# LJacksonPan/RaTrack

Measured on AMD Instinct MI355X. Metric: radar frame-pairs/sec (backbone forward, eval) at B=64,N=256 per GPU, higher is better.
Workload: dtype f32 (2xfp16 split MFMA: three fp16 products per fp32 product, fp32 accumulate, power-of-two scales per matrix and position); 1 GPU; Track4D.backbone forward, B=64 frame-pairs x N=256 points per GPU, S=512 centroids, eval-mode BN, random-init weights, hipGraph=True, batches in flight=4; global_batch=64, parallelism=replicas x1 (no collective on the forward path)

## Files before the change

### ratrack_amd/csrc/fused_split.hip

```cpp
#include "rtk_common.h"
#include "rtk_fused.h"
#include "split_mfma.h"

namespace {

#ifndef SP_NW
#define SP_NW 4
#endif
#ifndef SP_F
#define SP_F 32
#endif
constexpr int CV_F = 32;

__global__ __launch_bounds__(256) void pack_split_kernel(int cout, int cin, const float *__restrict__ w, int transposed, u4v *__restrict__ out,
                                                         float *__restrict__ inv_scale) {
    __shared__ unsigned s_m[4];
    float m = 0.f;
    const f4 *w4 = reinterpret_cast<const f4 *>(w);
    for (int i = threadIdx.x; i < cout * cin / 4; i += 256) {
        const f4 t = w4[i];
        m = __builtin_fmaxf(__builtin_fmaxf(m, __builtin_fabsf(t.x)), __builtin_fabsf(t.y));
        m = __builtin_fmaxf(__builtin_fmaxf(m, __builtin_fabsf(t.z)), __builtin_fabsf(t.w));
    }
    unsigned mb = __float_as_uint(m);
#pragma unroll
    for (int d = 32; d >= 1; d >>= 1) { const unsigned o = __shfl_xor(mb, d, 64); mb = o > mb ? o : mb; }
    if ((threadIdx.x & 63) == 0) s_m[threadIdx.x >> 6] = mb;
    __syncthreads();
    mb = max(max(s_m[0], s_m[1]), max(s_m[2], s_m[3]));
    const LaneScale sc = lane_scale_of(mb);
    if (blockIdx.x == 0 && threadIdx.x == 0) *inv_scale = sc.inv;
    const int VB = cout / 32, slot = blockIdx.x * 256 + threadIdx.x;
    if (slot >= (cin / 16) * VB * 64) return;
    const int lane = slot & 63, v = (slot >> 6) % VB, s = (slot >> 6) / VB, hh = lane >> 5, i = lane & 31;
    const int o = 32 * v + i, c0 = 32 * (s >> 1) + 16 * (s & 1) + 4 * hh;
    f4 x0, x1;
    if (transposed) {
#pragma unroll
        for (int r = 0; r < 4; ++r) { x0[r] = w[(size_t)(c0 + r) * cout + o]; x1[r] = w[(size_t)(c0 + 8 + r) * cout + o]; }
    } else {
        const float *row = w + (size_t)o * cin + c0;
        x0 = *reinterpret_cast<const f4 *>(row); x1 = *reinterpret_cast<const f4 *>(row + 8);
    }
    u4v b[2];
    split2(x0, x1, sc.s, b);
#pragma unroll
    for (int p = 0; p < 2; ++p) out[((size_t)(s * VB + v) * 2 + p) * 64 + lane] = b[p];
}

__device__ __forceinline__ f4 leaky_med4(f4 t, float inf) {
    const f4 u = t * 0.1f;
    return (f4){__builtin_amdgcn_fmed3f(t.x, u.x, inf), __builtin_amdgcn_fmed3f(t.y, u.y, inf), __builtin_amdgcn_fmed3f(t.z, u.z, inf),
                __builtin_amdgcn_fmed3f(t.w, u.w, inf)};
}
__device__ __forceinline__ f4 scale_bias4(f4 a, float c, f4 b) { return __builtin_elementwise_fma(a, (f4){c, c, c, c}, b); }

__global__ __launch_bounds__(64 * SP_NW) __attribute__((amdgpu_waves_per_eu(1, 1)))
void split_mlp2_kernel(int positions, const float *__restrict__ x, const f4 *__restrict__ blob, const float *__restrict__ wsc,
                       const float *__restrict__ bias1, const float *__restrict__ bias2, float *__restrict__ y) {
    const float kinf = rtk_hidden_inf();
    __shared__ __attribute__((aligned(16))) f4 s_w[2 * SP_F * 64];
    const int lane = threadIdx.x & 63, wave = __builtin_amdgcn_readfirstlane(threadIdx.x >> 6), hh = lane >> 5, col = lane & 31;
    constexpr int NF = 2 * SPLIT_NF;
    WStreamA<SP_NW, SP_F, NF> ws;
    ws.start_parts(blob, s_w, wave, lane);
    const float wi1 = ldc(wsc), wi2 = ldc(wsc + 1);
    const int tiles = (positions + 32 * SP_NW - 1) / (32 * SP_NW);
    for (int T = blockIdx.x; T < tiles; T += gridDim.x) {
        asm volatile("" ::: "memory");
        const long pos = (long)T * 32 * SP_NW + 32 * wave + col;
        const bool valid = pos < positions;
        const float *xr = x + (valid ? pos : (long)positions - 1) * 256 + 4 * hh;
        f4 h[32], bq[2][8];
#pragma unroll
        for (int i = 0; i < 32; ++i) h[i] = *reinterpret_cast<const f4 *>(xr + 8 * i);
        f16v acc[SPLIT_VB];
        LaneScale sc = lane_scale32(h);
        split_layer<0>(ws, h, sc.s, acc, BiasSide{bias1 + 4 * hh, bq});
        float c = sc.inv * wi1;
        split_epilogue(acc, bias1 + 4 * hh, bq, [&](int e, f4 a, f4 b) { h[e] = leaky_med4(scale_bias4(a, c, b), kinf); });
        sc = lane_scale32(h);
        split_layer<SPLIT_NF>(ws, h, sc.s, acc, BiasSide{bias2 + 4 * hh, bq});
        ws.sync();
        c = sc.inv * wi2;
        float *yr = y + pos * 256 + 4 * hh;
        split_epilogue(acc, bias2 + 4 * hh, bq, [&](int e, f4 a, f4 b) {
            if (valid) *reinterpret_cast<f4 *>(yr + 8 * e) = leaky_med4(scale_bias4(a, c, b), kinf);
        });
    }
    ws.finish();
}

struct CvSplitParams {
    int samples, n1, n2, gx;
    const float *xyz1, *xyz2;
    const int64_t *knn;
    const float *p1, *p2;
    const float *st;
    const float *wd;
    const f4 *blob;
    const float *wsc;
    const float *bias2, *bias3;
    WnSplit wn;
    float *out;
    int out_pitch;
    float *amax;
    float *sv1, *sv2, *sv3;
    uint2 *mk1, *mk2;
};

__device__ __forceinline__ void split_sign_masks(const f4 (&a)[32], uint2 (&m)[2]) {
    m[0] = m[1] = make_uint2(0u, 0u);
#pragma unroll
    for (int v = 0; v < SPLIT_VB; ++v)
#pragma unroll
        for (int q = 0; q < 4; ++q)
#pragma unroll
            for (int r = 0; r < 4; ++r) {
                const unsigned bit = (a[4 * v + q][r] > 0.f ? 1u : 0u) << (4 * ((2 * v + (q >> 1)) & 7) + r);
                if (v < 4) m[q & 1].x |= bit; else m[q & 1].y |= bit;
            }
}
__device__ __forceinline__ unsigned split_mask_bits(const uint2 (&m)[2], int v, int q) {
    return ((v < 4 ? m[q & 1].x : m[q & 1].y) >> (4 * ((2 * v + (q >> 1)) & 7))) & 15u;
}

__device__ __forceinline__ f4 *cv_at(float *base, unsigned byte_off) { return reinterpret_cast<f4 *>(reinterpret_cast<char *>(base) + byte_off); }
__device__ __forceinline__ const f4 *cv_at(const float *base, unsigned byte_off) {
    return reinterpret_cast<const f4 *>(reinterpret_cast<const char *>(base) + byte_off);
}

struct WnBlock {
    f16v bias;
    float w[4];
};
__device__ __forceinline__ WnBlock wn_block(const WnSplit &W, int v, int hh, int col) {
    WnBlock k;
    k.bias = split_bias(W.bc, v, hh);
    const int ch = 32 * v + col;
    const float *wr = W.wc + ((ch >> 4) * 64 + (ch & 15)) * 4;
#pragma unroll
    for (int st = 0; st < 4; ++st) {
        const int kk = 2 * st + hh;
        k.w[st] = ldc(wr + 64 * (kk >> 2) + (kk & 3));
    }
    return k;
}
__device__ __forceinline__ f16v wn_pre(const WnBlock &k, int hh, const float (&t2)[8]) {
    f16v w = k.bias;
#pragma unroll
    for (int st = 0; st < 4; ++st) w = mfma_f32x2(k.w[st], hh ? t2[2 * st + 1] : t2[2 * st], w);
    return w;
}

#ifndef CV_LDS_HIDDEN
#define CV_LDS_HIDDEN 1
#endif
#ifndef CV_WN_AHEAD
#define CV_WN_AHEAD 2
#endif
struct CvConsts {
    float wd[SPLIT_VB * 2 * 64];
    float wc[SPLIT_VB * 4 * 64];
    float bc[256], bias2[256], bias3[256];
#if CV_LDS_HIDDEN
    float hid[128];
#endif
};
static_assert(sizeof(CvConsts) == 15 * 1024 + (CV_LDS_HIDDEN ? 512 : 0), "4 + 8 + 3 KiB (+ the hidden layers)");
struct CvConstsFill {
    f4 wd, wc[2], bias;
    float hid;
};
__device__ __forceinline__ CvConstsFill cv_consts_load(const float *wd, const WnSplit &W, const float *bias2, const float *bias3, int wave, int lane) {
    CvConstsFill k;
    const int t = wave * 64 + lane;
    k.wd = ldc4(wd + 4 * t);
#pragma unroll
    for (int n = 0; n < 2; ++n) {
        const int u = 256 * n + t;
        k.wc[n] = ldc4(W.wc + (u >> 5) * 256 + ((u >> 4) & 1) * 64 + (u & 15) * 4);
    }
    const float *bs = wave == 0 ? W.bc : wave == 1 ? bias2 : bias3;
    k.bias = ldc4(bs + 4 * lane);
#if CV_LDS_HIDDEN
    {
        const int u = t < 32 ? 0 : t - 32, o = u >> 3, c = u & 7;
        const float *hs = t < 32 ? W.wa + 16 * (t >> 3) + (t & 7) : t < 96 ? W.wb + (16 * (c >> 2) + o) * 4 + (c & 3) : W.bb + (t < 104 ? t - 96 : 0);
        k.hid = ldc(hs);
    }
#endif
    return k;
}
__device__ __forceinline__ void cv_consts_store(CvConsts &C, const CvConstsFill &k, int wave, int lane) {
    const int t = wave * 64 + lane;
    {
        const int g = t >> 4, m = (t >> 2) & 3;
        *reinterpret_cast<f4 *>(C.wd + ((g >> 1) * 2 + (m >> 1)) * 64 + (m & 1) * 32 + (g & 1) * 16 + 4 * (t & 3)) = k.wd;
    }
#pragma unroll
    for (int n = 0; n < 2; ++n) {
        const int u = 256 * n + t, g = u >> 5, kq = (u >> 4) & 1, c15 = u & 15;
#pragma unroll
        for (int k3 = 0; k3 < 4; ++k3)
            C.wc[((g >> 1) * 4 + 2 * kq + (k3 >> 1)) * 64 + (k3 & 1) * 32 + (g & 1) * 16 + c15] = k.wc[n][k3];
    }
    if (wave < 3) *reinterpret_cast<f4 *>((wave == 0 ? C.bc : wave == 1 ? C.bias2 : C.bias3) + 4 * lane) = k.bias;
#if CV_LDS_HIDDEN
    if (t < 104) C.hid[t] = k.hid;
#endif
}
#if CV_LDS_HIDDEN
__device__ __forceinline__ void wn_hidden_lds(const CvConsts &C, float dx, float dy, float dz, float (&t2)[8]) {
    float t1[8];
#pragma unroll
    for (int o = 0; o < 8; ++o) {
        float a = __fmaf_rn(C.hid[o], dx, 0.f);
        a = __fmaf_rn(C.hid[8 + o], dy, a);
        a = __fmaf_rn(C.hid[16 + o], dz, a);
        t1[o] = fmaxf(__fadd_rn(a, C.hid[24 + o]), 0.f);
    }
#pragma unroll
    for (int o = 0; o < 8; ++o) {
        float a = C.hid[96 + o];
#pragma unroll
        for (int c = 0; c < 8; ++c) a = __fmaf_rn(C.hid[32 + 8 * o + c], t1[c], a);
        t2[o] = fmaxf(a, 0.f);
    }
}
#endif
__device__ __forceinline__ WnBlock wn_block_lds(const CvConsts &C, int v, int hh, int lane) {
    WnBlock k;
#pragma unroll
    for (int q = 0; q < 4; ++q) {
        const f4 t = *reinterpret_cast<const f4 *>(C.bc + 32 * v + 8 * q + 4 * hh);
        k.bias[4 * q] = t.x; k.bias[4 * q + 1] = t.y; k.bias[4 * q + 2] = t.z; k.bias[4 * q + 3] = t.w;
    }
#pragma unroll
    for (int st = 0; st < 4; ++st) k.w[st] = C.wc[(4 * v + st) * 64 + lane];
    return k;
}

constexpr int CV_ROWS_F4 = 32 * 32;
struct CvRowsRequest {
    const char *p2;
    f4 *rows;
    int nbrow;
    unsigned lanepart;
    int sub;
    __device__ __forceinline__ CvRowsRequest(const float *p2_, f4 *rows_, int nbrow_, int half, int lane)
        : p2(reinterpret_cast<const char *>(p2_)), rows(rows_), nbrow(nbrow_), lanepart(512u * half + (unsigned)(((lane & 31) ^ (lane >> 5)) << 4)), sub(lane >> 5) {}
    template <int T>
    __device__ __forceinline__ void one() const {
        const int r0 = __builtin_amdgcn_readlane(nbrow, 2 * T), r1 = __builtin_amdgcn_readlane(nbrow, 2 * T + 1);
        const unsigned off = ((unsigned)(sub ? r1 : r0) << 10) + (lanepart ^ (unsigned)(((2 * T) & 15) << 4));
        __builtin_amdgcn_global_load_lds((const __attribute__((address_space(1))) void *)(p2 + off),
                                         (__attribute__((address_space(3))) void *)(rows + T * 64), 16, 0, 0);
    }
    template <int... T>
    __device__ __forceinline__ void all(std::integer_sequence<int, T...>) const { (one<T>(), ...); }
};
template <int HALF>
__device__ __forceinline__ void cv_rows_request(const float *p2, int nbrow, f4 *rows, int lane) {
    asm volatile("s_waitcnt lgkmcnt(0)" ::: "memory");
    CvRowsRequest(p2, rows, nbrow, HALF, lane).all(std::make_integer_sequence<int, 16>{});
}
template <bool SAVE>
struct CvLayer2Side {
    StoreRowsSide st;
    CvRowsRequest rq;
    template <int GI>
    __device__ __forceinline__ void at(const f4 (&h)[32]) const {
        if constexpr (SAVE) st.template at<GI>(h);
        constexpr int per_chunk = CV_F / SPLIT_GF, ig = split_issue_groups(CV_F), g = GI % per_chunk, n = (GI / per_chunk) * ig + g;
        if constexpr (g < ig && 3 * n < 16) {
            rq.template one<3 * n>();
            if constexpr (3 * n + 1 < 16) rq.template one<3 * n + 1>();
            if constexpr (3 * n + 2 < 16) rq.template one<3 * n + 2>();
        }
    }
};
template <int HALF>
__device__ __forceinline__ void cv_rows_read(const f4 *rows, int col, int hh, f4 (&h)[32]) {
#pragma unroll
    for (int e = 0; e < 16; ++e) h[16 * HALF + e] = rows[col * 32 + ((2 * e + hh) ^ (col & 15))];
}
template <int K>
__device__ __forceinline__ f4 add_row_bcast(const f4 q, const f4 r) {
    f4 o;
    asm("s_nop 1\n"
        "v_add_f32_dpp %0, %4, %8 row_newbcast:%12 row_mask:0xf bank_mask:0xf\n"
        "v_add_f32_dpp %1, %5, %9 row_newbcast:%12 row_mask:0xf bank_mask:0xf\n"
        "v_add_f32_dpp %2, %6, %10 row_newbcast:%12 row_mask:0xf bank_mask:0xf\n"
        "v_add_f32_dpp %3, %7, %11 row_newbcast:%12 row_mask:0xf bank_mask:0xf"
        : "=&v"(o.x), "=&v"(o.y), "=&v"(o.z), "=&v"(o.w)
        : "v"(q.x), "v"(q.y), "v"(q.z), "v"(q.w), "v"(r.x), "v"(r.y), "v"(r.z), "v"(r.w), "n"(K));
    return o;
}
template <int K>
__device__ __forceinline__ f4 mul_row_bcast(const f4 q, const f4 r) {
    f4 o;
    asm("s_nop 1\n"
        "v_mul_f32_dpp %0, %4, %8 row_newbcast:%12 row_mask:0xf bank_mask:0xf\n"
        "v_mul_f32_dpp %1, %5, %9 row_newbcast:%12 row_mask:0xf bank_mask:0xf\n"
        "v_mul_f32_dpp %2, %6, %10 row_newbcast:%12 row_mask:0xf bank_mask:0xf\n"
        "v_mul_f32_dpp %3, %7, %11 row_newbcast:%12 row_mask:0xf bank_mask:0xf"
        : "=&v"(o.x), "=&v"(o.y), "=&v"(o.z), "=&v"(o.w)
        : "v"(q.x), "v"(q.y), "v"(q.z), "v"(q.w), "v"(r.x), "v"(r.y), "v"(r.z), "v"(r.w), "n"(K));
    return o;
}
__device__ __forceinline__ f4 add4_rn(const f4 a, const f4 b) {
    return (f4){__fadd_rn(a.x, b.x), __fadd_rn(a.y, b.y), __fadd_rn(a.z, b.z), __fadd_rn(a.w, b.w)};
}
template <int V0, int V1, bool LDSC>
__device__ __forceinline__ void cv_layer1_blocks(const CvSplitParams &P, const CvConsts &C, const f4 q0, const f4 q1, float b0, float b1, int hh, int col, float kinf, f4 (&h)[32]) {
    static_assert(V1 <= 8, "eight 32-channel blocks");
    auto block = [&](auto vc) {
        constexpr int v = decltype(vc)::value;
        f16v c;
        auto slot = [&](auto qc) {
            constexpr int q = decltype(qc)::value, e = 4 * v + q;
            const f4 t = add_row_bcast<e & 15>(e < 16 ? q0 : q1, h[e]);
            c[4 * q] = t.x; c[4 * q + 1] = t.y; c[4 * q + 2] = t.z; c[4 * q + 3] = t.w;
        };
        slot(std::integral_constant<int, 0>{}); slot(std::integral_constant<int, 1>{});
        slot(std::integral_constant<int, 2>{}); slot(std::integral_constant<int, 3>{});
        float a0, a1;
        if constexpr (LDSC) {
            a0 = C.wd[(2 * v) * 64 + 32 * hh + col]; a1 = C.wd[(2 * v + 1) * 64 + 32 * hh + col];
        } else {
            const int ch = 32 * v + col;
            const float *wr = P.wd + (ch >> 4) * 64 + (ch & 15);
            a0 = ldc(wr + 16 * hh); a1 = ldc(wr + 16 * (2 + hh));
        }
        c = mfma_f32x2(a0, b0, c);
        c = mfma_f32x2(a1, b1, c);
#pragma unroll
        for (int q = 0; q < 4; ++q) h[4 * v + q] = leaky_med4((f4){c[4 * q], c[4 * q + 1], c[4 * q + 2], c[4 * q + 3]}, kinf);
    };
    block(std::integral_constant<int, V0>{}); block(std::integral_constant<int, V0 + 1>{});
    block(std::integral_constant<int, V0 + 2>{}); block(std::integral_constant<int, V0 + 3>{});
}

#ifndef CV_FWD_VGPRS
#define CV_FWD_VGPRS 448
#endif
template <bool SAVE, bool LDSC = true>
__global__ __launch_bounds__(64 * SP_NW) __attribute__((amdgpu_waves_per_eu(1, 1), amdgpu_num_vgpr(CV_FWD_VGPRS)))
void cost_volume_split_kernel(const CvSplitParams P) {
    const float kinf = rtk_hidden_inf();
    __shared__ __attribute__((aligned(16))) f4 s_w[2 * CV_F * 64];
    __shared__ __attribute__((aligned(16))) f4 s_rows[SP_NW * CV_ROWS_F4];
    __shared__ __attribute__((aligned(16))) CvConsts s_c;
    const int lane = threadIdx.x & 63, wave = __builtin_amdgcn_readfirstlane(threadIdx.x >> 6), hh = lane >> 5, col = lane & 31, pp = col >> 4,
              j = col & 15;
    f4 *rows = s_rows + wave * CV_ROWS_F4;
    constexpr int PPW = 2 * SP_NW;
    const int groups = (P.n1 + PPW - 1) / PPW;
    const bool flat = P.gx > 0;
    const int xcd = blockIdx.x & 7, t0 = flat ? (int)(blockIdx.x >> 3) : (int)blockIdx.x, tstep = flat ? P.gx >> 3 : (int)gridDim.x;
    const int ntiles = flat ? (P.samples >> 3) * groups : groups;
    auto locate = [&](int t, int &b_, int &G_) {
        if (flat) { const int sk = t / groups; b_ = sk * 8 + xcd; G_ = t - sk * groups; }
        else { b_ = blockIdx.y; G_ = t; }
    };
    int b, bx;
    locate(t0 < ntiles ? t0 : 0, b, bx);
    WStreamA<SP_NW, CV_F, 2 * SPLIT_NF> ws;
    CvConstsFill cfill;
    if constexpr (LDSC) cfill = cv_consts_load(P.wd, P.wn, P.bias2, P.bias3, wave, lane);
    ws.start_parts(P.blob, s_w, wave, lane);
    if constexpr (LDSC) {
        cv_consts_store(s_c, cfill, wave, lane);
        __syncthreads();
    }
    const float *bias2 = (LDSC ? s_c.bias2 : P.bias2) + 4 * hh, *bias3 = (LDSC ? s_c.bias3 : P.bias3) + 4 * hh;
    auto wnb = [&](int v) {
        if constexpr (LDSC) return wn_block_lds(s_c, v, hh, lane);
        else return wn_block(P.wn, v, hh, col);
    };
    const float wi2 = ldc(P.wsc), wi3 = ldc(P.wsc + 1);
    int pt = bx * PPW + 2 * wave + pp;
    bool valid = pt < P.n1;
    long i = (long)b * P.n1 + (valid ? pt : P.n1 - 1);
    long nb = 0;
    float dx = 0.f, dy = 0.f, dz = 0.f;
    f4 q0 = {0.f, 0.f, 0.f, 0.f}, q1 = q0;
    if (t0 < ntiles) {
        nb = (long)b * P.n2 + (long)P.knn[i * 16 + j];
        cv_rows_request<0>(P.p2, (int)nb, rows, lane);
        q0 = ldc4(P.p1 + i * 256 + 4 * hh + 8 * j); q1 = ldc4(P.p1 + i * 256 + 4 * hh + 8 * (16 + j));
        if (P.st) { q0 = add4_rn(q0, ldc4(P.st + b * 256 + 4 * hh + 8 * j)); q1 = add4_rn(q1, ldc4(P.st + b * 256 + 4 * hh + 8 * (16 + j))); }
        dx = __fsub_rn(P.xyz2[nb * 3], P.xyz1[i * 3]); dy = __fsub_rn(P.xyz2[nb * 3 + 1], P.xyz1[i * 3 + 1]);
        dz = __fsub_rn(P.xyz2[nb * 3 + 2], P.xyz1[i * 3 + 2]);
    }
    for (int t = t0; t < ntiles; t += tstep) {
        asm volatile("" ::: "memory");
        const bool more = t + tstep < ntiles;
        int bn, Gn;
        locate(more ? t + tstep : t, bn, Gn);
        const int ptn = Gn * PPW + 2 * wave + pp;
        const bool validn = ptn < P.n1;
        const long in_ = (long)bn * P.n1 + (validn ? ptn : P.n1 - 1);
        long knn_next = 0;
        if (more) knn_next = (long)P.knn[in_ * 16 + j];
        f4 h[32];
        float t2[8];
        {
            const float b0 = hh ? dy : dx, b1 = hh ? 0.f : dz;
            cv_rows_read<0>(rows, col, hh, h);
            cv_rows_request<1>(P.p2, (int)nb, rows, lane);
            cv_layer1_blocks<0, 4, LDSC>(P, s_c, q0, q1, b0, b1, hh, col, kinf, h);
#if CV_LDS_HIDDEN
            if constexpr (LDSC && !SAVE) wn_hidden_lds(s_c, dx, dy, dz, t2);
            else
#endif
                wn_hidden(P.wn, dx, dy, dz, t2);
            __builtin_amdgcn_sched_barrier(0);
            cv_rows_read<1>(rows, col, hh, h);
            cv_layer1_blocks<4, 8, LDSC>(P, s_c, q0, q1, b0, b1, hh, col, kinf, h);
        }
        const long nbn = (long)bn * P.n2 + knn_next;
        const long pos = i * 16 + j;
        const unsigned ro = (unsigned)pos * 1024u + 16u * hh;
        if (SAVE && valid) {
            uint2 m[2];
            split_sign_masks(h, m);
            P.mk1[pos * 4 + hh] = m[0];
            P.mk1[pos * 4 + 2 + hh] = m[1];
        }
        f16v acc[SPLIT_VB];
        f4 bq[2][8];
        LaneScale sc = lane_scale32(h);
        if (SAVE && P.amax) tensor_amax_update(P.amax, sc.mb);
        split_layer<0>(ws, h, sc.s, acc, SidePair<CvLayer2Side<SAVE>, BiasSide>{{StoreRowsSide{P.sv1, ro, valid}, CvRowsRequest(P.p2, rows, (int)nbn, 0, lane)},
                                                                              BiasSide{bias2, bq}});
        float c = sc.inv * wi2;
        split_epilogue(acc, bias2, bq, [&](int e, f4 a, f4 b) { h[e] = leaky_med4(scale_bias4(a, c, b), kinf); });
        if (SAVE && valid) {
            uint2 m[2];
            split_sign_masks(h, m);
            P.mk2[pos * 4 + hh] = m[0];
            P.mk2[pos * 4 + 2 + hh] = m[1];
        }
        sc = lane_scale32(h);
        if (SAVE && P.amax) tensor_amax_update(P.amax + 1, sc.mb);
        if (SAVE) split_layer<SPLIT_NF>(ws, h, sc.s, acc, SidePair<StoreRowsSide, BiasSide>{StoreRowsSide{P.sv2, ro, valid}, BiasSide{bias3, bq}});
        else split_layer<SPLIT_NF>(ws, h, sc.s, acc, BiasSide{bias3, bq});
        ws.sync();
        c = sc.inv * wi3;
        split_epilogue(acc, bias3, bq, [&](int e, f4 a, f4 b) { h[e] = leaky_med4(scale_bias4(a, c, b), kinf); });
        if (SAVE && valid) {
#pragma unroll
            for (int e = 0; e < 32; ++e) *cv_at(P.sv3, ro + 32u * e) = h[e];
        }
        WnBlock wk = wnb(0);
        float *o = P.out + i * P.out_pitch + 4 * hh;
        f16v wpre = wn_pre(wk, hh, t2);
        constexpr bool ahead1 = LDSC && CV_WN_AHEAD == 1;
        if constexpr (!ahead1) wk = wnb(1);
        auto out_block = [&](int v) {
            const f16v w = wpre;
            if constexpr (ahead1) {
                if (v + 1 < SPLIT_VB) wk = wnb(v + 1);
            }
            if (v + 1 < SPLIT_VB) wpre = wn_pre(wk, hh, t2);
            if constexpr (!ahead1) {
                if (v + 2 < SPLIT_VB) wk = wnb(v + 2);
            }
            f4 r[4];
#pragma unroll
            for (int q = 0; q < 4; ++q)
#pragma unroll
                for (int e = 0; e < 4; ++e) r[q][e] = relu1(w[4 * q + e], kinf) * h[4 * v + q][e];
            const f4 t = row_sum16_transpose4(r[0], r[1], r[2], r[3]);
            if (valid && (j & 3) == 0) *reinterpret_cast<f4 *>(o + 32 * v + 8 * (2 * ((j >> 3) & 1) + ((j >> 2) & 1))) = t;
        };
        out_block(0);
        out_block(1);
        float cn[6] = {0.f, 0.f, 0.f, 0.f, 0.f, 0.f};
        f4 q0n = q0, q1n = q1, s0n = q0, s1n = q1;
        if (more) {
#pragma unroll
            for (int c = 0; c < 3; ++c) { cn[c] = ldc(P.xyz2 + nbn * 3 + c); cn[3 + c] = ldc(P.xyz1 + in_ * 3 + c); }
            q0n = ldc4(P.p1 + in_ * 256 + 4 * hh + 8 * j); q1n = ldc4(P.p1 + in_ * 256 + 4 * hh + 8 * (16 + j));
        }
        if (more && P.st) { s0n = ldc4(P.st + bn * 256 + 4 * hh + 8 * j); s1n = ldc4(P.st + bn * 256 + 4 * hh + 8 * (16 + j)); }
#pragma unroll
        for (int v = 2; v < SPLIT_VB; ++v) out_block(v);
        pt = ptn; valid = validn; i = in_; nb = nbn; q0 = q0n; q1 = q1n;
        if (P.st) { q0 = add4_rn(q0n, s0n); q1 = add4_rn(q1n, s1n); }
        dx = __fsub_rn(cn[0], cn[3]); dy = __fsub_rn(cn[1], cn[4]); dz = __fsub_rn(cn[2], cn[5]);
    }
    ws.finish();
}

struct CvSplitBwdParams {
    CvSplitParams f;
    const float *dout;
    int dout_pitch;
    const float *a3;
    const uint2 *mk1, *mk2;
    float *dz1, *dz2, *dz3, *dq3, *d4, *dp1, *dpd, *dt2, *dbrows;
};

__device__ __forceinline__ f4 leaky_grad_bits4(f4 d, unsigned bits) {
    return (f4){(bits & 1u) ? d.x : 0.1f * d.x, (bits & 2u) ? d.y : 0.1f * d.y, (bits & 4u) ? d.z : 0.1f * d.z, (bits & 8u) ? d.w : 0.1f * d.w};
}

__global__ __launch_bounds__(64 * SP_NW) __attribute__((amdgpu_waves_per_eu(1, 1))) void cost_volume_bwd_split_kernel(const CvSplitBwdParams Q) {
    const float kinf = rtk_hidden_inf();
    __shared__ __attribute__((aligned(16))) f4 s_w[2 * SP_F * 64];
    __shared__ float s_wct[128 * 64];
    const CvSplitParams &P = Q.f;
    const int lane = threadIdx.x & 63, wave = __builtin_amdgcn_readfirstlane(threadIdx.x >> 6), hh = lane >> 5, col = lane & 31, pp = col >> 4,
              j = col & 15;
    const int jq = 2 * ((j >> 3) & 1) + ((j >> 2) & 1);
    for (int e = threadIdx.x; e < 128 * 64; e += 64 * SP_NW) {
        const int l = e & 63, st = e >> 6, o = l & 31, ch = 32 * (st >> 4) + 8 * ((st >> 2) & 3) + 4 * (l >> 5) + (st & 3);
        s_wct[e] = o < 8 ? P.wn.wc[((ch >> 4) * 64 + (o >> 2) * 16 + (ch & 15)) * 4 + (o & 3)] : 0.f;
    }
    int b, bx, nbx;
    rtk_decode_block(P.gx, b, bx, nbx);
    constexpr int PPW = 2 * SP_NW;
    const int groups = (P.n1 + PPW - 1) / PPW;
    WStreamA<SP_NW, SP_F, 2 * SPLIT_NF> ws;
    ws.start_parts(P.blob, s_w, wave, lane);
    const float wi3 = ldc(P.wsc), wi2 = ldc(P.wsc + 1);
    int pt = bx * PPW + 2 * wave + pp;
    bool valid = pt < P.n1;
    long i = (long)b * P.n1 + (valid ? pt : P.n1 - 1);
    float dx = 0.f, dy = 0.f, dz = 0.f;
    if (bx < groups) {
        const long nb = (long)b * P.n2 + (long)P.knn[i * 16 + j];
        dx = __fsub_rn(P.xyz2[nb * 3], P.xyz1[i * 3]); dy = __fsub_rn(P.xyz2[nb * 3 + 1], P.xyz1[i * 3 + 1]);
        dz = __fsub_rn(P.xyz2[nb * 3 + 2], P.xyz1[i * 3 + 2]);
    }
    for (int G = bx; G < groups; G += nbx) {
        asm volatile("" ::: "memory");
        const long pos = i * 16 + j;
        const unsigned ro = (unsigned)pos * 1024u + 16u * hh;
        if (valid && hh == 0) *reinterpret_cast<f4 *>(Q.d4 + pos * 4) = (f4){dx, dy, dz, 1.0f};
        uint2 m2[2] = {Q.mk2[pos * 4 + hh], Q.mk2[pos * 4 + 2 + hh]}, m1[2] = {Q.mk1[pos * 4 + hh], Q.mk1[pos * 4 + 2 + hh]};
        f4 h[32];
#pragma unroll
        for (int e = 0; e < 32; ++e) h[e] = *cv_at(Q.a3, ro + 32u * e);
        float t2[8];
        WnBlock wk = wn_block(P.wn, 0, hh, col);
        const float *dor = Q.dout + i * Q.dout_pitch + 4 * hh;
        const f4 dq0 = ldc4(dor + 8 * j), dq1 = ldc4(dor + 8 * (16 + j));
        wn_hidden(P.wn, dx, dy, dz, t2);
        f16v dt2;
#pragma unroll
        for (int e = 0; e < 16; ++e) dt2[e] = 0.f;
        f16v wpre = wn_pre(wk, hh, t2);
        wk = wn_block(P.wn, 1, hh, col);
        auto block_a = [&](auto vc) {
            constexpr int v = decltype(vc)::value;
            const f16v w = wpre;
            if constexpr (v + 1 < SPLIT_VB) wpre = wn_pre(wk, hh, t2);
            if constexpr (v + 2 < SPLIT_VB) wk = wn_block(P.wn, v + 2, hh, col);
            f4 zs[4];
            auto slot = [&](auto qc) {
                constexpr int q = decltype(qc)::value, e = 4 * v + q;
                const f4 a = h[e];
                f4 wv;
#pragma unroll
                for (int r = 0; r < 4; ++r) wv[r] = relu1(w[4 * q + r], kinf);
                const f4 da = mul_row_bcast<e & 15>(e < 16 ? dq0 : dq1, a);
                const f4 t = mul_row_bcast<e & 15>(e < 16 ? dq0 : dq1, wv);
                f4 qq, z;
#pragma unroll
                for (int r = 0; r < 4; ++r) {
                    qq[r] = wv[r] > 0.f ? da[r] : 0.f;
                    z[r] = a[r] > 0.f ? t[r] : 0.1f * t[r];
                    dt2 = mfma_f32x2(s_wct[(16 * v + 4 * q + r) * 64 + lane], qq[r], dt2);
                }
                h[e] = z;
                zs[q] = z;
                if (valid) *cv_at(Q.dq3, ro + 32u * e) = qq;
            };
            slot(std::integral_constant<int, 0>{}); slot(std::integral_constant<int, 1>{});
            slot(std::integral_constant<int, 2>{}); slot(std::integral_constant<int, 3>{});
            if (Q.dbrows) {
                const f4 r = row_sum16_transpose4(zs[0], zs[1], zs[2], zs[3]);
                if (valid && (j & 3) == 0) *reinterpret_cast<f4 *>(Q.dbrows + i * 512 + 32 * v + 8 * jq + 4 * hh) = r;
            }
        };
        block_a(std::integral_constant<int, 0>{}); block_a(std::integral_constant<int, 1>{}); block_a(std::integral_constant<int, 2>{});
        block_a(std::integral_constant<int, 3>{}); block_a(std::integral_constant<int, 4>{}); block_a(std::integral_constant<int, 5>{});
        block_a(std::integral_constant<int, 6>{}); block_a(std::integral_constant<int, 7>{});
        if (valid) *reinterpret_cast<f4 *>(Q.dt2 + pos * 8 + 4 * hh) = (f4){dt2[0], dt2[1], dt2[2], dt2[3]};
        f16v acc[SPLIT_VB];
        LaneScale sc = lane_scale32(h);
        if (P.amax) tensor_amax_update(P.amax, sc.mb);
        split_layer<0>(ws, h, sc.s, acc, StoreRowsSide{Q.dz3, ro, valid});
        float c = sc.inv * wi3;
#pragma unroll
        for (int v = 0; v < SPLIT_VB; ++v) {
#pragma unroll
            for (int q = 0; q < 4; ++q) h[4 * v + q] = leaky_grad_bits4(acc_slot(acc, 4 * v + q) * c, split_mask_bits(m2, v, q));
            if (Q.dbrows) {
                const f4 r = row_sum16_transpose4(h[4 * v], h[4 * v + 1], h[4 * v + 2], h[4 * v + 3]);
                if (valid && (j & 3) == 0) *reinterpret_cast<f4 *>(Q.dbrows + i * 512 + 256 + 32 * v + 8 * jq + 4 * hh) = r;
            }
        }
        sc = lane_scale32(h);
        if (P.amax) tensor_amax_update(P.amax + 1, sc.mb);
        split_layer<SPLIT_NF>(ws, h, sc.s, acc, StoreRowsSide{Q.dz2, ro, valid});
        ws.sync();
        c = sc.inv * wi2;
        const int Gn = G + nbx;
        const bool more = Gn < groups;
        const int ptn = Gn * PPW + 2 * wave + pp;
        const bool validn = ptn < P.n1;
        const long in_ = (long)b * P.n1 + (validn ? ptn : P.n1 - 1);
        long knn_next = 0;
        if (more) knn_next = (long)P.knn[in_ * 16 + j];
        float dxn = 0.f, dyn = 0.f, dzn = 0.f;
        float *dpr = Q.dp1 + i * 256 + 4 * hh;
        float *dpd = Q.dpd + i * 768 + 4 * hh;
#pragma unroll
        for (int v = 0; v < SPLIT_VB; ++v) {
            if (v == 2 && more) {
                const long nbn = (long)b * P.n2 + knn_next;
                dxn = __fsub_rn(P.xyz2[nbn * 3], P.xyz1[in_ * 3]); dyn = __fsub_rn(P.xyz2[nbn * 3 + 1], P.xyz1[in_ * 3 + 1]);
                dzn = __fsub_rn(P.xyz2[nbn * 3 + 2], P.xyz1[in_ * 3 + 2]);
            }
            f4 r[4];
#pragma unroll
            for (int q = 0; q < 4; ++q) {
                r[q] = leaky_grad_bits4(acc_slot(acc, 4 * v + q) * c, split_mask_bits(m1, v, q));
                if (valid) *cv_at(Q.dz1, ro + 32u * (4 * v + q)) = r[q];
            }
            const f4 s0 = row_sum16_transpose4(r[0], r[1], r[2], r[3]);
            const f4 sx = row_sum16_transpose4(r[0] * dx, r[1] * dx, r[2] * dx, r[3] * dx);
            const f4 sy = row_sum16_transpose4(r[0] * dy, r[1] * dy, r[2] * dy, r[3] * dy);
            const f4 sz = row_sum16_transpose4(r[0] * dz, r[1] * dz, r[2] * dz, r[3] * dz);
            if (valid && (j & 3) == 0) {
                *reinterpret_cast<f4 *>(dpr + 32 * v + 8 * jq) = s0;
                *reinterpret_cast<f4 *>(dpd + 32 * v + 8 * jq) = sx;
                *reinterpret_cast<f4 *>(dpd + 256 + 32 * v + 8 * jq) = sy;
                *reinterpret_cast<f4 *>(dpd + 512 + 32 * v + 8 * jq) = sz;
            }
        }
        pt = ptn; valid = validn; i = in_; dx = dxn; dy = dyn; dz = dzn;
    }
    ws.finish();
}

struct SaSplitParams {
    int samples, n, npoint, gx;
    const float *xyz, *new_xyz;
    const int *idx;
    const float *q;
    int q_pitch;
    const float *w1;
    const f4 *image;
    const float *wsc;
    const float *bias2;
    float *out;
    int out_pitch, out_offset;
    const int *src_nuniq, *dst_nuniq;
};

#ifndef SA_SPLIT_WAVES
#define SA_SPLIT_WAVES 5
#endif
#ifndef SA_WGS_TARGET
#define SA_WGS_TARGET 1024
#endif
template <int NS, int C1>
__global__ __launch_bounds__(256, SA_SPLIT_WAVES) void sa_scale_split_kernel(const SaSplitParams P) {
    constexpr int KS = C1 / 16, VB1 = C1 / 32, NFR = KS * 2 * 2, CPT = 32 / NS;
    static_assert(RTK_BALL_TAIL_ROWS % CPT == 0, "a tile of CPT centroids must not reach past the ball tables' zero tail");
    const float kinf = rtk_hidden_inf();
    __shared__ __attribute__((aligned(16))) f4 s_img[NFR * 64];
    const int lane = threadIdx.x & 63, hh = lane >> 5, col = lane & 31, pp = col / NS, slot = col % NS;
    int b, bx, nbx;
    rtk_decode_block(P.gx, b, bx, nbx);
    const int dst_e = P.dst_nuniq ? __builtin_amdgcn_readfirstlane(P.dst_nuniq[b]) : P.npoint;
    const int live_c = min(dst_e, P.npoint);
    const int live_units = (live_c + CPT - 1) / CPT;
    if (bx * 4 >= live_units) return;
    for (int i = threadIdx.x; i < NFR * 64; i += blockDim.x) s_img[i] = P.image[i];
    __syncthreads();
    const int src_e = P.src_nuniq ? P.src_nuniq[b] : 0x7fffffff;
    const float winv = ldc(P.wsc);
    for (int unit = bx * 4 + (threadIdx.x >> 6); unit < live_units; unit += nbx * 4) {
        int cl = unit * CPT + pp;
        const bool valid = cl < live_c;
        if (!valid) cl = live_c - 1;
        const int c = b * P.npoint + cl;
        const int id = P.idx[(long)c * NS + slot];
        const long src = (long)b * P.n + id;
        const float dx = __fsub_rn(P.xyz[src * 3], P.new_xyz[(long)c * 3]), dy = __fsub_rn(P.xyz[src * 3 + 1], P.new_xyz[(long)c * 3 + 1]),
                    dz = __fsub_rn(P.xyz[src * 3 + 2], P.new_xyz[(long)c * 3 + 2]);
        const float *qrow = P.q + ((long)b * P.n + (id < src_e ? id : 0)) * P.q_pitch + 4 * hh;
        const float b0 = hh ? dy : dx, b1 = hh ? 1.0f : dz;
        f4 h[4 * VB1];
#pragma unroll
        for (int v = 0; v < VB1; ++v) {
            f16v a;
#pragma unroll
            for (int q = 0; q < 4; ++q) {
                const f4 t = *reinterpret_cast<const f4 *>(qrow + 32 * v + 8 * q);
                a[4 * q] = t.x; a[4 * q + 1] = t.y; a[4 * q + 2] = t.z; a[4 * q + 3] = t.w;
            }
            const int ch = 32 * v + col;
            const float *wr = P.w1 + (ch >> 4) * 64 + (ch & 15);
            a = mfma_f32x2(wr[16 * hh], b0, a);
            a = mfma_f32x2(wr[16 * (2 + hh)], b1, a);
#pragma unroll
            for (int q = 0; q < 4; ++q) h[4 * v + q] = relu_med4((f4){a[4 * q], a[4 * q + 1], a[4 * q + 2], a[4 * q + 3]}, kinf);
        }
        const LaneScale sc = lane_scale32(h);
        const float cs = sc.inv * winv;
        f16v acc[2];
#pragma unroll
        for (int v = 0; v < 2; ++v)
#pragma unroll
            for (int e = 0; e < 16; ++e) acc[v][e] = 0.f;
#pragma unroll
        for (int s = 0; s < KS; ++s) {
            u4v bp[2];
            split2(h[2 * s], h[2 * s + 1], sc.s, bp);
            u4v fr[2][2];
#pragma unroll
            for (int v = 0; v < 2; ++v)
#pragma unroll
                for (int p = 0; p < 2; ++p) fr[v][p] = __builtin_bit_cast(u4v, s_img[((s * 2 + v) * 2 + p) * 64 + lane]);
#define RTK_SA_MM(pa, pb) acc[0] = mfma_h(fr[0][pa], bp[pb], acc[0]); acc[1] = mfma_h(fr[1][pa], bp[pb], acc[1]);
            RTK_SA_MM(1, 0) RTK_SA_MM(0, 1) RTK_SA_MM(0, 0)
#undef RTK_SA_MM
        }
        f4 m[2][4];
#pragma unroll
        for (int v = 0; v < 2; ++v)
#pragma unroll
            for (int q = 0; q < 4; ++q)
                m[v][q] = scale_bias4((f4){acc[v][4 * q], acc[v][4 * q + 1], acc[v][4 * q + 2], acc[v][4 * q + 3]}, cs,
                                      *reinterpret_cast<const f4 *>(P.bias2 + 32 * v + 8 * q + 4 * hh));
        const int qo = 2 * ((col >> 3) & 1) + ((col >> 2) & 1);
        float *o = P.out + (long)c * P.out_pitch + P.out_offset + 4 * hh + 8 * qo;
        if constexpr (NS == 32) {
            f4 t[4];
#pragma unroll
            for (int q = 0; q < 4; ++q) t[q] = wave_max_pair16(m[0][q], m[1][q], kinf);
            const f4 r = relu_med4(row_max16_transpose4(t[0], t[1], t[2], t[3]), kinf);
            if (valid && (col & 3) == 0) *reinterpret_cast<f4 *>(o + 32 * ((col >> 4) & 1)) = r;
        } else {
#pragma unroll
            for (int v = 0; v < 2; ++v) {
                const f4 r = relu_med4(row_max16_transpose4(m[v][0], m[v][1], m[v][2], m[v][3]), kinf);
                if (valid && (col & 3) == 0) *reinterpret_cast<f4 *>(o + 32 * v) = r;
            }
        }
    }
}

}

extern "C" int rtk_pack_split_layer(int cout, int cin, const float *w, int transposed, void *image, float *inv_scale, rtk_stream_t stream) {
    RTK_REQUIRE(cout > 0 && cin > 0 && cout % 32 == 0 && cin % 32 == 0 && w && image && inv_scale, "pack_split_layer: bad arguments");
    RTK_REQUIRE((long)cout * cin <= (1L << 22), "pack_split_layer: more than 2^22 weights (every workgroup scans the matrix for its scale)");
    const int slots = (cin / 16) * (cout / 32) * 64;
    pack_split_kernel<<<(slots + 255) / 256, 256, 0, (hipStream_t)stream>>>(cout, cin, w, transposed, (u4v *)image, inv_scale);
    RTK_CHECK_LAUNCH("pack_split_layer");
    return RTK_OK;
}

extern "C" int rtk_split_mlp2(int positions, const float *x, const void *images, const float *image_scales, const float *bias1,
                              const float *bias2, float *y, rtk_stream_t stream) {
    RTK_REQUIRE(positions > 0 && x && images && image_scales && bias1 && bias2 && y, "split_mlp2: bad arguments");
    const int tiles = (positions + 32 * SP_NW - 1) / (32 * SP_NW);
    split_mlp2_kernel<<<tiles < 256 ? tiles : 256, 64 * SP_NW, 0, (hipStream_t)stream>>>(positions, x, (const f4 *)images, image_scales, bias1, bias2, y);
    RTK_CHECK_LAUNCH("split_mlp2");
    return RTK_OK;
}

static int cv_split_fill(const char *who, CvSplitParams &P, int samples, int n1, int n2, const float *xyz1, const float *xyz2,
                         const int64_t *knn_idx, const void *split_images, const float *image_scales, const rtk_layer_t *wn, dim3 &grid) {
    RTK_REQUIRE(samples > 0 && samples <= 65535 && n1 > 0 && n2 >= 16 && xyz1 && xyz2 && knn_idx && split_images && image_scales,
                "%s: bad arguments", who);
    RTK_REQUIRE(wn && wn[0].w_packed && wn[1].w_packed && wn[2].w_packed && wn[1].bias && wn[2].bias && wn[1].cin16 == 1 &&
                wn[1].cout16 == 1 && wn[2].cin16 == 1 && wn[2].cout16 == 16, "%s: bad WeightNet layers", who);
    P.samples = samples; P.n1 = n1; P.n2 = n2;
    P.xyz1 = xyz1; P.xyz2 = xyz2; P.knn = knn_idx;
    P.blob = reinterpret_cast<const f4 *>(split_images);
    P.wsc = image_scales;
    P.wn.wa = wn[0].w_packed; P.wn.wb = wn[1].w_packed; P.wn.wc = wn[2].w_packed; P.wn.bb = wn[1].bias; P.wn.bc = wn[2].bias;
    P.p1 = P.p2 = P.st = P.wd = P.bias2 = P.bias3 = nullptr;
    P.out = nullptr; P.out_pitch = 0; P.sv1 = P.sv2 = P.sv3 = nullptr; P.mk1 = P.mk2 = nullptr; P.amax = nullptr;
    const int groups = (n1 + 2 * SP_NW - 1) / (2 * SP_NW);
    int gx = 256 / samples;
    if (gx < 1) gx = 1;
    if (gx > groups) gx = groups;
    P.gx = samples % 8 == 0 ? gx : 0;
    grid = P.gx ? dim3(gx * samples) : dim3(gx, samples);
    return RTK_OK;
}

static int cu_count() {
    int dev = 0, n = 0;
    if (hipGetDevice(&dev) != hipSuccess || hipDeviceGetAttribute(&n, hipDeviceAttributeMultiprocessorCount, dev) != hipSuccess || n < 8) return 256;
    return n;
}

static int cv_split_forward(const char *who, int samples, int n1, int n2, const float *xyz1, const float *xyz2, const int64_t *knn_idx,
                            const float *p1, const float *p2, const float *wd_packed, const void *split_images, const float *image_scales,
                            const float *bias2, const float *bias3, const rtk_layer_t *wn, float *out, int out_pitch, float *a1, float *a2,
                            float *a3, void *mask1, void *mask2, float *amax, int workgroups, rtk_stream_t stream,
                            const float *sample_term = nullptr, bool global_consts = false) {
    CvSplitParams P;
    dim3 grid;
    if (cv_split_fill(who, P, samples, n1, n2, xyz1, xyz2, knn_idx, split_images, image_scales, wn, grid) != RTK_OK) return RTK_ERR_INVALID;
    RTK_REQUIRE(p1 && p2 && wd_packed && bias2 && bias3 && out, "%s: bad arguments", who);
    RTK_REQUIRE((double)samples * n2 <= 4194304.0, "%s: more than 2^22 rows in p2 (32-bit byte offsets of the row requests): split the batch", who);
    RTK_REQUIRE(out_pitch % 4 == 0 && out_pitch >= 256, "%s: bad out_pitch", who);
    const bool save = a1 != nullptr;
    RTK_REQUIRE(!save || ((double)samples * n1 * 16.0 * 1024.0 < 4294967296.0), "%s: more than 4 GiB per saved activation (32-bit row "
                "offsets): split the batch", who);
    P.p1 = p1; P.p2 = p2; P.st = sample_term; P.wd = wd_packed; P.bias2 = bias2; P.bias3 = bias3; P.out = out; P.out_pitch = out_pitch;
    P.sv1 = a1; P.sv2 = a2; P.sv3 = a3; P.mk1 = (uint2 *)mask1; P.mk2 = (uint2 *)mask2; P.amax = amax;
    if (samples % 8 == 0) {
        const int tiles_x = (samples / 8) * ((n1 + 2 * SP_NW - 1) / (2 * SP_NW));
        int per_xcd = (workgroups > 0 ? workgroups : cu_count()) / 8;
        if (per_xcd < 1) per_xcd = 1;
        if (per_xcd > tiles_x) per_xcd = tiles_x;
        P.gx = 8 * per_xcd;
        grid = dim3(P.gx);
    }
    if (save) cost_volume_split_kernel<true><<<grid, 64 * SP_NW, 0, (hipStream_t)stream>>>(P);
    else if (global_consts) cost_volume_split_kernel<false, false><<<grid, 64 * SP_NW, 0, (hipStream_t)stream>>>(P);
    else cost_volume_split_kernel<false><<<grid, 64 * SP_NW, 0, (hipStream_t)stream>>>(P);
    RTK_CHECK_LAUNCH(who);
    return RTK_OK;
}

extern "C" int rtk_cost_volume_split(int samples, int n1, int n2, const float *xyz1, const float *xyz2, const int64_t *knn_idx,
                                     const float *p1, const float *p2, const float *wd_packed, const void *split_images,
                                     const float *image_scales, const float *bias2, const float *bias3, const rtk_layer_t *wn, float *out,
                                     int out_pitch, rtk_stream_t stream) {
    return cv_split_forward("cost_volume_split", samples, n1, n2, xyz1, xyz2, knn_idx, p1, p2, wd_packed, split_images, image_scales, bias2, bias3,
                            wn, out, out_pitch, nullptr, nullptr, nullptr, nullptr, nullptr, nullptr, 0, stream);
}

extern "C" int rtk_cost_volume_split_shared(int samples, int n1, int n2, const float *xyz1, const float *xyz2, const int64_t *knn_idx,
                                            const float *p1, const float *p2, const float *wd_packed, const void *split_images,
                                            const float *image_scales, const float *bias2, const float *bias3, const rtk_layer_t *wn,
                                            float *out, int out_pitch, int workgroups, rtk_stream_t stream) {
    RTK_REQUIRE(workgroups >= 0, "cost_volume_split_shared: workgroups = %d", workgroups);
    return cv_split_forward("cost_volume_split_shared", samples, n1, n2, xyz1, xyz2, knn_idx, p1, p2, wd_packed, split_images, image_scales,
                            bias2, bias3, wn, out, out_pitch, nullptr, nullptr, nullptr, nullptr, nullptr, nullptr, workgroups, stream);
}

extern "C" int rtk_cost_volume_split_gconst(int samples, int n1, int n2, const float *xyz1, const float *xyz2, const int64_t *knn_idx,
                                            const float *p1, const float *p2, const float *wd_packed, const void *split_images,
                                            const float *image_scales, const float *bias2, const float *bias3, const rtk_layer_t *wn,
                                            float *out, int out_pitch, int workgroups, rtk_stream_t stream) {
    RTK_REQUIRE(workgroups >= 0, "cost_volume_split_gconst: workgroups = %d", workgroups);
    return cv_split_forward("cost_volume_split_gconst", samples, n1, n2, xyz1, xyz2, knn_idx, p1, p2, wd_packed, split_images, image_scales,
                            bias2, bias3, wn, out, out_pitch, nullptr, nullptr, nullptr, nullptr, nullptr, nullptr, workgroups, stream, nullptr, true);
}

extern "C" int rtk_cost_volume_split_term(int samples, int n1, int n2, const float *xyz1, const float *xyz2, const int64_t *knn_idx,
                                          const float *p1, const float *p2, const float *sample_term, const float *wd_packed,
                                          const void *split_images, const float *image_scales, const float *bias2, const float *bias3,
                                          const rtk_layer_t *wn, float *out, int out_pitch, int workgroups, rtk_stream_t stream) {
    RTK_REQUIRE(workgroups >= 0 && sample_term, "cost_volume_split_term: workgroups = %d, sample_term = %p", workgroups, (const void *)sample_term);
    return cv_split_forward("cost_volume_split_term", samples, n1, n2, xyz1, xyz2, knn_idx, p1, p2, wd_packed, split_images, image_scales,
                            bias2, bias3, wn, out, out_pitch, nullptr, nullptr, nullptr, nullptr, nullptr, nullptr, workgroups, stream, sample_term);
}

extern "C" int rtk_cost_volume_split_train(int samples, int n1, int n2, const float *xyz1, const float *xyz2, const int64_t *knn_idx,
                                           const float *p1, const float *p2, const float *wd_packed, const void *split_images,
                                           const float *image_scales, const float *bias2, const float *bias3, const rtk_layer_t *wn,
                                           float *out, int out_pitch, float *a1, float *a2, float *a3, void *mask1, void *mask2,
                                           float *act_amax, rtk_stream_t stream) {
    RTK_REQUIRE(a1 && a2 && a3 && mask1 && mask2, "cost_volume_split_train: null activation buffer");
    return cv_split_forward("cost_volume_split_train", samples, n1, n2, xyz1, xyz2, knn_idx, p1, p2, wd_packed, split_images, image_scales,
                            bias2, bias3, wn, out, out_pitch, a1, a2, a3, mask1, mask2, act_amax, 0, stream);
}

extern "C" int rtk_cost_volume_bwd_split(int samples, int n1, int n2, const float *xyz1, const float *xyz2, const int64_t *knn_idx,
                                         const void *split_images_t, const float *image_scales_t, const rtk_layer_t *wn, const float *dout,
                                         int dout_pitch,
                                         const float *a3, const void *mask1, const void *mask2, float *dz1, float *dz2, float *dz3,
                                         float *dq3, float *d4, float *dp1, float *dpd, float *dt2, float *dbias_rows,
                                         float *dz_amax, rtk_stream_t stream) {
    CvSplitBwdParams Q;
    dim3 grid;
    if (cv_split_fill("cost_volume_bwd_split", Q.f, samples, n1, n2, xyz1, xyz2, knn_idx, split_images_t, image_scales_t, wn, grid) != RTK_OK)
        return RTK_ERR_INVALID;
    RTK_REQUIRE(dout && mask1 && mask2 && a3 && dz1 && dz2 && dz3 && dq3 && d4 && dp1 && dpd && dt2, "cost_volume_bwd_split: bad arguments");
    RTK_REQUIRE((double)samples * n1 * 16.0 * 1024.0 < 4294967296.0, "cost_volume_bwd_split: more than 4 GiB per (position, 256) tensor "
                "(32-bit row offsets): split the batch");
    RTK_REQUIRE(dout_pitch % 4 == 0 && dout_pitch >= 256, "cost_volume_bwd_split: bad dout_pitch");
    Q.dout = dout; Q.dout_pitch = dout_pitch; Q.a3 = a3; Q.mk1 = (const uint2 *)mask1; Q.mk2 = (const uint2 *)mask2;
    Q.dz1 = dz1; Q.dz2 = dz2; Q.dz3 = dz3; Q.dq3 = dq3; Q.d4 = d4; Q.dp1 = dp1; Q.dpd = dpd; Q.dt2 = dt2; Q.dbrows = dbias_rows;
    Q.f.amax = dz_amax;
    cost_volume_bwd_split_kernel<<<grid, 64 * SP_NW, 0, (hipStream_t)stream>>>(Q);
    RTK_CHECK_LAUNCH("cost_volume_bwd_split");
    return RTK_OK;
}

extern "C" int rtk_sa_scale_split(int samples, int n, int npoint, int nsample, const float *xyz, const float *new_xyz, const int *idx,
                                  const float *q, int q_pitch, int c1, const float *w1xyz_packed, const void *split_image,
                                  const float *image_scale, const float *bias2, float *out, int out_pitch, int out_offset,
                                  const int *src_nuniq, const int *dst_nuniq, rtk_stream_t stream) {
    RTK_REQUIRE(samples > 0 && n > 0 && npoint > 0 && xyz && new_xyz && idx && q && w1xyz_packed && split_image && image_scale && bias2 && out,
                "sa_scale_split: bad arguments");
    RTK_REQUIRE(q_pitch % 4 == 0 && out_pitch % 4 == 0 && out_offset % 4 == 0, "sa_scale_split: pitches/offset must be multiples of 4");
    RTK_REQUIRE((long)samples * npoint * nsample < 0x7fffffffL && (long)samples * n < 0x7fffffffL && samples <= 65535,
                "sa_scale_split: problem too large for 32-bit indexing");
    SaSplitParams P;
    P.samples = samples; P.n = n; P.npoint = npoint;
    P.xyz = xyz; P.new_xyz = new_xyz; P.idx = idx; P.q = q; P.q_pitch = q_pitch; P.w1 = w1xyz_packed;
    P.image = reinterpret_cast<const f4 *>(split_image); P.wsc = image_scale; P.bias2 = bias2;
    P.out = out; P.out_pitch = out_pitch; P.out_offset = out_offset; P.src_nuniq = src_nuniq; P.dst_nuniq = dst_nuniq;
    const int units = (npoint + 32 / nsample - 1) / (32 / nsample);
    int bx = (units + 3) / 4;
    while ((long)bx * samples > SA_WGS_TARGET && bx > 1) bx = (bx + 1) / 2;
    P.gx = samples % 8 == 0 ? bx : 0;
    const dim3 blocks = P.gx ? dim3(bx * samples) : dim3(bx, samples);
    hipStream_t s = (hipStream_t)stream;
    if (nsample == 32 && c1 == 64) sa_scale_split_kernel<32, 64><<<blocks, 256, 0, s>>>(P);
    else if (nsample == 16 && c1 == 64) sa_scale_split_kernel<16, 64><<<blocks, 256, 0, s>>>(P);
    else if (nsample == 16 && c1 == 32) sa_scale_split_kernel<16, 32><<<blocks, 256, 0, s>>>(P);
    else {
        rtk_set_error("sa_scale_split: no kernel instance for nsample=%d, %d -> 64 channels", nsample, c1);
        return RTK_ERR_UNSUPPORTED;
    }
    RTK_CHECK_LAUNCH("sa_scale_split");
    return RTK_OK;
}
```

Before: 108,600 frame-pairs/s.

## Stream LDS-resident conv biases through a small register ring in epilogue

```diff
diff --git a/ratrack_amd/csrc/fused_split.hip b/ratrack_amd/csrc/fused_split.hip
--- a/ratrack_amd/csrc/fused_split.hip
+++ b/ratrack_amd/csrc/fused_split.hip
@@ -157,7 +157,7 @@
 #define CV_LDS_HIDDEN 1
 #endif
 #ifndef CV_WN_AHEAD
-#define CV_WN_AHEAD 2
+#define CV_WN_AHEAD 1
 #endif
 struct CvConsts {
     float wd[SPLIT_VB * 2 * 64];
@@ -239,6 +239,36 @@
 #pragma unroll
     for (int st = 0; st < 4; ++st) k.w[st] = C.wc[(4 * v + st) * 64 + lane];
     return k;
+}
+
+#ifndef CV_BIAS_AHEAD
+#define CV_BIAS_AHEAD 4
+#endif
+struct BiasLdsSide {
+    const float *bias;
+    f4 (&br)[CV_BIAS_AHEAD];
+    template <int GI>
+    __device__ __forceinline__ void at(const f4 (&)[32]) const {
+        constexpr int NG = SPLIT_KS * (SPLIT_VB / 2), H = CV_BIAS_AHEAD / 2;
+        if constexpr (GI >= NG - 2) {
+#pragma unroll
+            for (int e = H * (GI - (NG - 2)); e < H * (GI - (NG - 2) + 1); ++e) br[e] = bias_slot(bias, e);
+        }
+    }
+};
+template <class Emit>
+__device__ __forceinline__ void split_epilogue_lds(const f16v (&acc)[SPLIT_VB], const float *bias4hh, f4 (&br)[CV_BIAS_AHEAD], Emit &&emit) {
+    static_assert(CV_BIAS_AHEAD % 2 == 0 && 8 % CV_BIAS_AHEAD == 0, "a ring of 2, 4 or 8 slots");
+#pragma unroll
+    for (int k = 0; k < 4; ++k) {
+#pragma unroll
+        for (int e = 8 * k; e < 8 * k + 8; ++e) {
+            const f4 b = br[e % CV_BIAS_AHEAD];
+            if (e + CV_BIAS_AHEAD < 32) br[e % CV_BIAS_AHEAD] = bias_slot(bias4hh, e + CV_BIAS_AHEAD);
+            emit(e, acc_slot(acc, e), b);
+        }
+        __builtin_amdgcn_sched_barrier(0);
+    }
 }
 
 constexpr int CV_ROWS_F4 = 32 * 32;
@@ -430,13 +460,19 @@
             P.mk1[pos * 4 + 2 + hh] = m[1];
         }
         f16v acc[SPLIT_VB];
-        f4 bq[2][8];
+        constexpr bool lds_bias = LDSC && !SAVE;
+        f4 bq[lds_bias ? 1 : 2][lds_bias ? CV_BIAS_AHEAD : 8];
         LaneScale sc = lane_scale32(h);
         if (SAVE && P.amax) tensor_amax_update(P.amax, sc.mb);
-        split_layer<0>(ws, h, sc.s, acc, SidePair<CvLayer2Side<SAVE>, BiasSide>{{StoreRowsSide{P.sv1, ro, valid}, CvRowsRequest(P.p2, rows, (int)nbn, 0, lane)},
-                                                                              BiasSide{bias2, bq}});
+        if constexpr (lds_bias)
+            split_layer<0>(ws, h, sc.s, acc, SidePair<CvLayer2Side<SAVE>, BiasLdsSide>{{StoreRowsSide{P.sv1, ro, valid}, CvRowsRequest(P.p2, rows, (int)nbn, 0, lane)},
+                                                                                     BiasLdsSide{bias2, bq[0]}});
+        else
+            split_layer<0>(ws, h, sc.s, acc, SidePair<CvLayer2Side<SAVE>, BiasSide>{{StoreRowsSide{P.sv1, ro, valid}, CvRowsRequest(P.p2, rows, (int)nbn, 0, lane)},
+                                                                                  BiasSide{bias2, bq}});
         float c = sc.inv * wi2;
-        split_epilogue(acc, bias2, bq, [&](int e, f4 a, f4 b) { h[e] = leaky_med4(scale_bias4(a, c, b), kinf); });
+        if constexpr (lds_bias) split_epilogue_lds(acc, bias2, bq[0], [&](int e, f4 a, f4 b) { h[e] = leaky_med4(scale_bias4(a, c, b), kinf); });
+        else split_epilogue(acc, bias2, bq, [&](int e, f4 a, f4 b) { h[e] = leaky_med4(scale_bias4(a, c, b), kinf); });
         if (SAVE && valid) {
             uint2 m[2];
             split_sign_masks(h, m);
@@ -445,11 +481,13 @@
         }
         sc = lane_scale32(h);
         if (SAVE && P.amax) tensor_amax_update(P.amax + 1, sc.mb);
-        if (SAVE) split_layer<SPLIT_NF>(ws, h, sc.s, acc, SidePair<StoreRowsSide, BiasSide>{StoreRowsSide{P.sv2, ro, valid}, BiasSide{bias3, bq}});
+        if constexpr (lds_bias) split_layer<SPLIT_NF>(ws, h, sc.s, acc, BiasLdsSide{bias3, bq[0]});
+        else if constexpr (SAVE) split_layer<SPLIT_NF>(ws, h, sc.s, acc, SidePair<StoreRowsSide, BiasSide>{StoreRowsSide{P.sv2, ro, valid}, BiasSide{bias3, bq}});
         else split_layer<SPLIT_NF>(ws, h, sc.s, acc, BiasSide{bias3, bq});
         ws.sync();
         c = sc.inv * wi3;
-        split_epilogue(acc, bias3, bq, [&](int e, f4 a, f4 b) { h[e] = leaky_med4(scale_bias4(a, c, b), kinf); });
+        if constexpr (lds_bias) split_epilogue_lds(acc, bias3, bq[0], [&](int e, f4 a, f4 b) { h[e] = leaky_med4(scale_bias4(a, c, b), kinf); });
+        else split_epilogue(acc, bias3, bq, [&](int e, f4 a, f4 b) { h[e] = leaky_med4(scale_bias4(a, c, b), kinf); });
         if (SAVE && valid) {
 #pragma unroll
             for (int e = 0; e < 32; ++e) *cv_at(P.sv3, ro + 32u * e) = h[e];
@@ -457,7 +495,7 @@
         WnBlock wk = wnb(0);
         float *o = P.out + i * P.out_pitch + 4 * hh;
         f16v wpre = wn_pre(wk, hh, t2);
-        constexpr bool ahead1 = LDSC && CV_WN_AHEAD == 1;
+        constexpr bool ahead1 = LDSC && !SAVE && CV_WN_AHEAD == 1;
         if constexpr (!ahead1) wk = wnb(1);
         auto out_block = [&](int v) {
             const f16v w = wpre;
```

Result: no change. 109,600 frame-pairs/s, median of 6 (+0.9%).
